# JohannesErnst/WeaSAL

Measured on AMD Instinct MI355X. Metric: points/sec fwd+bwd KPFCNN on DALES spheres; achieved HBM GB/s on KPConv gather, higher is better.
Workload: dtype f32; 1 GPU; DALES_PseudoLabel KP-FCNN, in_radius=10m, 50k pts/sphere, batch=8, fp32, step = GPU pyramid + fwd + loss + bwd + SGD; contrast_loss term included (trainer_PseudoLabel.py:204-208); pyramid of the next batch overlapped on a second stream; parallelism=dp1, dist_world_size=1, allreduce_bytes=0

## Files before the change

### weasal_amd/csrc/contrast_mfma.hip

```cpp
#include "ws_common.h"

namespace {

typedef float f32x4v __attribute__((ext_vector_type(4)));
constexpr int CM_SMAX = 1024;
constexpr float CM_TMIN = 0.023f, CM_TMAX = 1.0e26f;
constexpr int CM_CP = 17;

__device__ __forceinline__ void lds_order()
{
    asm volatile("s_waitcnt lgkmcnt(0)" ::: "memory");
    __builtin_amdgcn_wave_barrier();
}

constexpr int CF_TILES = 2;
constexpr int CF_WAVES = 8;

template <int NS>
__global__ __launch_bounds__(512) void contrast_fwd_mfma_kernel(const float* __restrict__ on, int64_t n, int c,
                                                                 const float* __restrict__ xs, int s,
                                                                 const int64_t* __restrict__ slc_idx, const uint8_t* __restrict__ certain,
                                                                 const int64_t* __restrict__ lbl, float temperature, float eps,
                                                                 float* __restrict__ loss, float* __restrict__ rowmax,
                                                                 float* __restrict__ den, float* __restrict__ npos)
{
    __shared__ float sx[CM_SMAX][4 * NS];
    __shared__ int sidx[CM_SMAX], stag[CM_SMAX];
    const int ncol = (s + 15) & ~15;
    for (int e = threadIdx.x; e < ncol * 4 * NS; e += 512) {
        const int j = e / (4 * NS), cc = e % (4 * NS);
        sx[j][cc] = (j < s && cc < c) ? xs[(int64_t)j * c + cc] : 0.0f;
    }
    for (int j = threadIdx.x; j < ncol; j += 512) {
        const int64_t p = j < s ? slc_idx[j] : 0;
        sidx[j] = j < s ? (int)p : -1;
        stag[j] = j < s ? (((int)lbl[p] << 1) | (certain[p] ? 1 : 0)) : -2;
    }
    __syncthreads();
    const int wave = threadIdx.x >> 6, lane = threadIdx.x & 63;
    const int i = lane & 15, kk = lane >> 4;
    const float inv_t = 1.0f / temperature;
    for (int t = 0; t < CF_TILES; ++t) {
        const int64_t p0 = (((int64_t)blockIdx.x * CF_WAVES + wave) * CF_TILES + t) * 16;
        if (p0 >= n) break;
        float a[NS];
        {
            const int64_t pi = p0 + i < n ? p0 + i : n - 1;
#pragma unroll
            for (int st = 0; st < NS; ++st) a[st] = (4 * st + kk) < c ? on[pi * c + 4 * st + kk] : 0.0f;
        }
        int ptag[4], pidx[4];
        float m[4], E[4], P[4], S[4];
#pragma unroll
        for (int r = 0; r < 4; ++r) {
            const int64_t p = p0 + 4 * kk + r;
            const int64_t pc = p < n ? p : n - 1;
            pidx[r] = (int)p;
            ptag[r] = ((int)lbl[pc] << 1) | (certain[pc] ? 1 : 0);
            m[r] = -3.0e38f; E[r] = 0.0f; P[r] = 0.0f; S[r] = 0.0f;
        }
        for (int c0 = 0; c0 < ncol; c0 += 16) {
            f32x4v d = f32x4v{0.f, 0.f, 0.f, 0.f};
#pragma unroll
            for (int st = 0; st < NS; ++st) d = __builtin_amdgcn_mfma_f32_16x16x4f32(a[st], sx[c0 + i][4 * st + kk], d, 0, 0, 0);
            const int tg = stag[c0 + i], sid = sidx[c0 + i];
            const bool colok = tg != -2;
#pragma unroll
            for (int r = 0; r < 4; ++r) {
                const float mul = d[r] * inv_t;
                m[r] = colok ? fmaxf(m[r], mul) : m[r];
                const bool use = colok && sid != pidx[r] && ((tg ^ ptag[r]) & 1) == 0;
                const bool pos = use && tg == ptag[r];
                E[r] += use ? __expf(mul - inv_t) : 0.0f;
                P[r] += pos ? 1.0f : 0.0f;
                S[r] += pos ? mul : 0.0f;
            }
        }
#pragma unroll
        for (int r = 0; r < 4; ++r) {
#pragma unroll
            for (int o = 1; o < 16; o <<= 1) {
                m[r] = fmaxf(m[r], __shfl_xor(m[r], o, 64));
                E[r] += __shfl_xor(E[r], o, 64);
                P[r] += __shfl_xor(P[r], o, 64);
                S[r] += __shfl_xor(S[r], o, 64);
            }
            const int64_t p = p0 + 4 * kk + r;
            if (i == 0 && p < n) {
                const float Er = E[r] * __expf(inv_t - m[r]);
                const float dd = Er + eps;
                loss[p] = -temperature * (((S[r] - P[r] * m[r]) - P[r] * logf(dd)) / (P[r] + 1e-12f));
                rowmax[p] = m[r];
                den[p] = dd;
                npos[p] = P[r];
            }
        }
    }
}

constexpr int CB_TILES = 4;
constexpr int CB_WLD = 17;

template <int NS>
__global__ __launch_bounds__(256) void contrast_bwd_mfma_kernel(const float* __restrict__ on, int64_t n, int c,
                                                                 const float* __restrict__ xs, int s,
                                                                 const int64_t* __restrict__ slc_idx, const uint8_t* __restrict__ certain,
                                                                 const int64_t* __restrict__ lbl, float temperature,
                                                                 const float* __restrict__ rowmax, const float* __restrict__ den,
                                                                 const float* __restrict__ npos, const float* __restrict__ g,
                                                                 float* __restrict__ d_on, float* __restrict__ partial)
{
    __shared__ float po_all[4][16 * CB_TILES][CM_CP];
    __shared__ float4 pst_all[4][16 * CB_TILES];
    __shared__ int ptg_all[4][16 * CB_TILES];
    __shared__ float wt_all[4][16 * CB_WLD];
    __shared__ float ds_all[4][16][16];
    const int wave = threadIdx.x >> 6, lane = threadIdx.x & 63;
    const int i = lane & 15, kk = lane >> 4;
    float (*po)[CM_CP] = po_all[wave];
    float4* pst = pst_all[wave];
    int* ptg = ptg_all[wave];
    float* wt = wt_all[wave];
    const int64_t pw0 = ((int64_t)blockIdx.x * 4 + wave) * (16 * CB_TILES);
    const float inv_t = 1.0f / temperature;
    for (int e = lane; e < 16 * CB_TILES * CM_CP; e += 64) {
        const int r = e / CM_CP, cc = e % CM_CP;
        const int64_t p = pw0 + r;
        po[r][cc] = (p < n && cc < c) ? on[p * c + cc] : 0.0f;
    }
    for (int r = lane; r < 16 * CB_TILES; r += 64) {
        const int64_t p = pw0 + r;
        const bool live = p < n;
        const float P = live ? npos[p] : 0.0f;
        pst[r] = make_float4(live ? rowmax[p] : 0.0f, P, live ? 1.0f / den[p] : 0.0f,
                             live ? g[p] * (-temperature / (P + 1e-12f)) / temperature : 0.0f);
        ptg[r] = live ? (((int)lbl[p] << 1) | (certain[p] ? 1 : 0)) : -4;
    }
    lds_order();
    f32x4v don[CB_TILES];
#pragma unroll
    for (int t = 0; t < CB_TILES; ++t) don[t] = f32x4v{0.f, 0.f, 0.f, 0.f};
    const int ncol = (s + 15) & ~15;
    for (int c0 = 0; c0 < ncol; c0 += 16) {
        float b1[NS], b2[4];
        const int col = c0 + i;
        const int colc = col < s ? col : s - 1;
#pragma unroll
        for (int st = 0; st < NS; ++st) b1[st] = (col < s && 4 * st + kk < c) ? xs[(int64_t)colc * c + 4 * st + kk] : 0.0f;
#pragma unroll
        for (int st = 0; st < 4; ++st) {
            const int cj = c0 + 4 * st + kk;
            b2[st] = (cj < s && i < c) ? xs[(int64_t)cj * c + i] : 0.0f;
        }
        const int64_t sp = slc_idx[colc];
        const int sid = col < s ? (int)sp : -1;
        const int tg = col < s ? (((int)lbl[sp] << 1) | (certain[sp] ? 1 : 0)) : -2;
        f32x4v dsa = f32x4v{0.f, 0.f, 0.f, 0.f};
#pragma unroll
        for (int t = 0; t < CB_TILES; ++t) {
            f32x4v d = f32x4v{0.f, 0.f, 0.f, 0.f};
#pragma unroll
            for (int st = 0; st < NS; ++st) d = __builtin_amdgcn_mfma_f32_16x16x4f32(po[16 * t + i][4 * st + kk], b1[st], d, 0, 0, 0);
            lds_order();
#pragma unroll
            for (int r = 0; r < 4; ++r) {
                const int pr = 16 * t + 4 * kk + r;
                const float4 st4 = pst[pr];
                const int ptag = ptg[pr];
                const float lg = d[r] * inv_t - st4.x;
                const bool use = tg != -2 && ptag != -4 && sid != (int)(pw0 + pr) && ((tg ^ ptag) & 1) == 0;
                const bool pos = use && tg == ptag;
                const float w = st4.w * ((pos ? 1.0f : 0.0f) - (use ? st4.y * __expf(lg) * st4.z : 0.0f));
                wt[(4 * kk + r) * CB_WLD + i] = w;
            }
            lds_order();
#pragma unroll
            for (int st = 0; st < 4; ++st) {
                don[t] = __builtin_amdgcn_mfma_f32_16x16x4f32(wt[i * CB_WLD + 4 * st + kk], b2[st], don[t], 0, 0, 0);
                dsa = __builtin_amdgcn_mfma_f32_16x16x4f32(po[16 * t + 4 * st + kk][i], wt[(4 * st + kk) * CB_WLD + i], dsa, 0, 0, 0);
            }
        }
#pragma unroll
        for (int r = 0; r < 4; ++r) ds_all[wave][4 * kk + r][i] = dsa[r];
        __syncthreads();
        {
            const int ch = threadIdx.x >> 4, cj = threadIdx.x & 15;
            if (ch < c && c0 + cj < s)
                partial[((int64_t)blockIdx.x * s + c0 + cj) * c + ch] = (ds_all[0][ch][cj] + ds_all[1][ch][cj]) + (ds_all[2][ch][cj] + ds_all[3][ch][cj]);
        }
        __syncthreads();
    }
#pragma unroll
    for (int t = 0; t < CB_TILES; ++t)
#pragma unroll
        for (int r = 0; r < 4; ++r) {
            const int64_t p = pw0 + 16 * t + 4 * kk + r;
            if (p < n && i < c) d_on[p * c + i] = don[t][r];
        }
}

__global__ __launch_bounds__(1024) void contrast_reduce2_kernel(const float* __restrict__ partial, int64_t elems, int chunks,
                                                                 float* __restrict__ out)
{
    __shared__ float red[32][33];
    const int el = threadIdx.x & 31, cl = threadIdx.x >> 5;
    const int64_t e = (int64_t)blockIdx.x * 32 + el;
    float sacc = 0.0f;
    if (e < elems)
        for (int cidx = cl; cidx < chunks; cidx += 32) sacc += partial[(int64_t)cidx * elems + e];
    red[cl][el] = sacc;
    __syncthreads();
    for (int o = 16; o > 0; o >>= 1) {
        if (cl < o) red[cl][el] += red[cl + o][el];
        __syncthreads();
    }
    if (cl == 0 && e < elems) out[e] = red[0][el];
}

}

extern "C" {

int ws_contrast_rows_fwd(const float* on, int64_t n, int32_t c, const float* xs, int32_t s, const int64_t* slc_idx,
                         const uint8_t* certain, const int64_t* lbl, float temperature, float eps, float* loss,
                         float* rowmax, float* den, float* npos, void* stream)
{
    WS_REQUIRE(n >= 0 && c >= 1 && s >= 1, "bad sizes n=%lld c=%d s=%d", (long long)n, c, s);
    if (c > 16 || s > CM_SMAX) return ws_fail(WS_ERR_UNSUPPORTED, "contrast rows: c=%d (<= 16) s=%d (<= %d)", c, s, CM_SMAX);
    WS_REQUIRE(temperature >= CM_TMIN && temperature <= CM_TMAX, "contrast rows: temperature %g outside [%g, %g]", (double)temperature, (double)CM_TMIN, (double)CM_TMAX);
    WS_REQUIRE(n < (1ll << 31), "n exceeds int32");
    if (n == 0) return WS_OK;
    WS_REQUIRE(on && xs && slc_idx && certain && lbl && loss && rowmax && den && npos, "NULL argument");
    hipStream_t st = (hipStream_t)stream;
    const unsigned grid = (unsigned)ws_ceil_div(n, CF_WAVES * CF_TILES * 16);
    if (c <= 4) contrast_fwd_mfma_kernel<1><<<grid, 64 * CF_WAVES, 0, st>>>(on, n, c, xs, s, slc_idx, certain, lbl, temperature, eps, loss, rowmax, den, npos);
    else if (c <= 8) contrast_fwd_mfma_kernel<2><<<grid, 64 * CF_WAVES, 0, st>>>(on, n, c, xs, s, slc_idx, certain, lbl, temperature, eps, loss, rowmax, den, npos);
    else if (c <= 12) contrast_fwd_mfma_kernel<3><<<grid, 64 * CF_WAVES, 0, st>>>(on, n, c, xs, s, slc_idx, certain, lbl, temperature, eps, loss, rowmax, den, npos);
    else contrast_fwd_mfma_kernel<4><<<grid, 64 * CF_WAVES, 0, st>>>(on, n, c, xs, s, slc_idx, certain, lbl, temperature, eps, loss, rowmax, den, npos);
    WS_LAUNCH_CHECK();
    return WS_OK;
}

int64_t ws_contrast_rows_bwd_scratch_bytes(int64_t n, int32_t c, int32_t s)
{
    return ws_ceil_div(n > 0 ? n : 1, 4 * CB_TILES * 16) * (int64_t)s * c * (int64_t)sizeof(float);
}

int ws_contrast_rows_bwd(const float* on, int64_t n, int32_t c, const float* xs, int32_t s, const int64_t* slc_idx,
                         const uint8_t* certain, const int64_t* lbl, float temperature, const float* rowmax,
                         const float* den, const float* npos, const float* g, float* d_on, float* d_xs, void* scratch,
                         void* stream)
{
    WS_REQUIRE(n >= 0 && c >= 1 && s >= 1, "bad sizes n=%lld c=%d s=%d", (long long)n, c, s);
    if (c > 16 || s > CM_SMAX) return ws_fail(WS_ERR_UNSUPPORTED, "contrast rows: c=%d (<= 16) s=%d (<= %d)", c, s, CM_SMAX);
    WS_REQUIRE(temperature >= CM_TMIN && temperature <= CM_TMAX, "contrast rows: temperature %g outside [%g, %g]", (double)temperature, (double)CM_TMIN, (double)CM_TMAX);
    WS_REQUIRE(d_xs, "NULL argument");
    hipStream_t st = (hipStream_t)stream;
    if (n == 0) {
        WS_HIP(hipMemsetAsync(d_xs, 0, sizeof(float) * (size_t)s * c, st));
        return WS_OK;
    }
    WS_REQUIRE(on && xs && slc_idx && certain && lbl && rowmax && den && npos && g && d_on && scratch, "NULL argument");
    const int chunks = (int)ws_ceil_div(n, 4 * CB_TILES * 16);
    float* partial = chunks == 1 ? d_xs : (float*)scratch;
#define WS_CBM(NSV) contrast_bwd_mfma_kernel<NSV><<<chunks, 256, 0, st>>>(on, n, c, xs, s, slc_idx, certain, lbl, temperature, rowmax, den, npos, g, d_on, partial)
    if (c <= 4) WS_CBM(1);
    else if (c <= 8) WS_CBM(2);
    else if (c <= 12) WS_CBM(3);
    else WS_CBM(4);
#undef WS_CBM
    WS_LAUNCH_CHECK();
    if (chunks > 1) {
        const int64_t elems = (int64_t)s * c;
        contrast_reduce2_kernel<<<(unsigned)ws_ceil_div(elems, 32), 1024, 0, st>>>(partial, elems, chunks, d_xs);
        WS_LAUNCH_CHECK();
    }
    return WS_OK;
}

}
```

Baseline: 32.61 million points/s.

## Partition contrast slice columns by certainty to skip masked work in forward kernel

Result: no change. 32.63 million points/s (median of 2 runs) (+0.1%).

```diff
diff --git a/weasal_amd/csrc/contrast_mfma.hip b/weasal_amd/csrc/contrast_mfma.hip
--- a/weasal_amd/csrc/contrast_mfma.hip
+++ b/weasal_amd/csrc/contrast_mfma.hip
@@ -4,8 +4,11 @@
 
 typedef float f32x4v __attribute__((ext_vector_type(4)));
 constexpr int CM_SMAX = 1024;
+constexpr int CM_STAB = CM_SMAX + 16;
 constexpr float CM_TMIN = 0.023f, CM_TMAX = 1.0e26f;
 constexpr int CM_CP = 17;
+constexpr int CM_NTAG = 64;
+constexpr float CM_LOG2E = 1.44269504088896340736f;
 
 __device__ __forceinline__ void lds_order()
 {
@@ -13,35 +16,145 @@
     __builtin_amdgcn_wave_barrier();
 }
 
+struct SliceGroups { int nc, nc16, ntot; };
+
+template <int NT, typename Mark>
+__device__ __forceinline__ SliceGroups stage_slice_meta(int s, const int64_t* __restrict__ slc_idx, const uint8_t* __restrict__ certain,
+                                                         const int64_t* __restrict__ lbl, int* sorig, int* stag, int* sidx,
+                                                         int* chunk_cnt, Mark mark)
+{
+    static_assert(CM_SMAX % NT == 0 && NT % 64 == 0, "whole 64-column chunks per round");
+    constexpr int ROUNDS = CM_SMAX / NT, NCHUNK = CM_SMAX / 64;
+    const int lane = threadIdx.x & 63;
+    const unsigned long long below = (1ull << lane) - 1ull;
+    int pnt[ROUNDS], tag[ROUNDS];
+    unsigned long long cmask[ROUNDS];
+#pragma unroll
+    for (int r = 0; r < ROUNDS; ++r) {
+        const int j = r * NT + (int)threadIdx.x;
+        const bool live = j < s;
+        const int64_t p = live ? slc_idx[j] : 0;
+        pnt[r] = (int)p;
+        tag[r] = live ? (((int)lbl[p] << 1) | (certain[p] ? 1 : 0)) : -2;
+        cmask[r] = __ballot(live && (tag[r] & 1));
+        if (lane == 0) chunk_cnt[j >> 6] = __popcll(cmask[r]);
+    }
+    __syncthreads();
+    int nc = 0;
+#pragma unroll
+    for (int k = 0; k < NCHUNK; ++k) nc += chunk_cnt[k];
+    nc = __builtin_amdgcn_readfirstlane(nc);
+    SliceGroups gr;
+    gr.nc = nc;
+    gr.nc16 = (nc + 15) & ~15;
+    const int nu = s - nc;
+    gr.ntot = gr.nc16 + ((nu + 15) & ~15);
+#pragma unroll
+    for (int r = 0; r < ROUNDS; ++r) {
+        const int j = r * NT + (int)threadIdx.x;
+        if (j < s) {
+            const int k = j >> 6;
+            int before = 0;
+            for (int q = 0; q < k; ++q) before += chunk_cnt[q];
+            const int cb = __popcll(cmask[r] & below);
+            const int pos = (tag[r] & 1) ? before + cb : gr.nc16 + (64 * k - before) + (lane - cb);
+            sorig[pos] = j;
+            stag[pos] = tag[r];
+            sidx[pos] = pnt[r];
+            mark(pos, pnt[r], tag[r]);
+        }
+    }
+    if (threadIdx.x < 32) {
+        const int q = threadIdx.x & 15;
+        const int pos = threadIdx.x < 16 ? nc + q : gr.nc16 + nu + q;
+        if (pos < (threadIdx.x < 16 ? gr.nc16 : gr.ntot)) {
+            sorig[pos] = -1;
+            stag[pos] = -2;
+            sidx[pos] = -1;
+        }
+    }
+    __syncthreads();
+    return gr;
+}
+
 constexpr int CF_TILES = 2;
 constexpr int CF_WAVES = 8;
+static_assert(CF_TILES * CF_WAVES <= 32, "one self bit per point tile of the workgroup");
+
+template <bool FAST>
+__device__ __forceinline__ void contrast_fwd_tile(const f32x4v d, const int tg, const int sid, const int (&ptag)[4], const int (&pidx)[4],
+                                                  const float k1, const float top, float (&m)[4], float (&E)[4], float (&P)[4], float (&S)[4])
+{
+    const bool colok = tg != -2;
+#pragma unroll
+    for (int r = 0; r < 4; ++r) {
+        const float e = __builtin_amdgcn_exp2f(__builtin_fmaf(d[r], k1, -k1));
+        if (FAST) {
+            m[r] = __builtin_amdgcn_fmed3f(m[r], d[r], top);
+            E[r] += e;
+            S[r] += tg == ptag[r] ? d[r] : 0.0f;
+        } else {
+            m[r] = colok ? fmaxf(m[r], d[r]) : m[r];
+            const bool use = colok && sid != pidx[r] && ((tg ^ ptag[r]) & 1) == 0;
+            const bool pos = use && tg == ptag[r];
+            E[r] += use ? e : 0.0f;
+            P[r] += pos ? 1.0f : 0.0f;
+            S[r] += pos ? d[r] : 0.0f;
+        }
+    }
+}
 
 template <int NS>
-__global__ __launch_bounds__(512) void contrast_fwd_mfma_kernel(const float* __restrict__ on, int64_t n, int c,
+__global__ __launch_bounds__(64 * CF_WAVES) void contrast_fwd_mfma_kernel(const float* __restrict__ on, int64_t n, int c,
                                                                  const float* __restrict__ xs, int s,
                                                                  const int64_t* __restrict__ slc_idx, const uint8_t* __restrict__ certain,
                                                                  const int64_t* __restrict__ lbl, float temperature, float eps,
                                                                  float* __restrict__ loss, float* __restrict__ rowmax,
                                                                  float* __restrict__ den, float* __restrict__ npos)
 {
-    __shared__ float sx[CM_SMAX][4 * NS];
-    __shared__ int sidx[CM_SMAX], stag[CM_SMAX];
-    const int ncol = (s + 15) & ~15;
-    for (int e = threadIdx.x; e < ncol * 4 * NS; e += 512) {
-        const int j = e / (4 * NS), cc = e % (4 * NS);
-        sx[j][cc] = (j < s && cc < c) ? xs[(int64_t)j * c + cc] : 0.0f;
-    }
-    for (int j = threadIdx.x; j < ncol; j += 512) {
-        const int64_t p = j < s ? slc_idx[j] : 0;
-        sidx[j] = j < s ? (int)p : -1;
-        stag[j] = j < s ? (((int)lbl[p] << 1) | (certain[p] ? 1 : 0)) : -2;
+    constexpr int NT = 64 * CF_WAVES;
+    __shared__ float sx[CM_STAB][4 * NS];
+    __shared__ int sidx[CM_STAB], stag[CM_STAB], sorig[CM_STAB];
+    __shared__ int chunk_cnt[CM_SMAX / 64], tagcnt[CM_NTAG], flags[2];
+    if (threadIdx.x < CM_NTAG) tagcnt[threadIdx.x] = 0;
+    if (threadIdx.x < 2) flags[threadIdx.x] = 0;
+    const int64_t blk0 = (int64_t)blockIdx.x * (CF_WAVES * CF_TILES * 16);
+    const SliceGroups gr = stage_slice_meta<NT>(s, slc_idx, certain, lbl, sorig, stag, sidx, chunk_cnt,
+        [&](int, int pnt, int tag) {
+            const int64_t rel = (int64_t)pnt - blk0;
+            if (rel >= 0 && rel < CF_WAVES * CF_TILES * 16) atomicOr(&flags[0], 1 << (int)(rel >> 4));
+            if (tag >= 0 && tag < CM_NTAG) atomicAdd(&tagcnt[tag], 1);
+            else atomicOr(&flags[1], 1);
+        });
+    const int total = gr.ntot * 4 * NS;
+    for (int e0 = threadIdx.x; e0 < total; e0 += NT * 8) {
+        float v[8];
+#pragma unroll
+        for (int u = 0; u < 8; ++u) {
+            const int e = e0 + u * NT < total ? e0 + u * NT : total - 1;
+            const int j = e / (4 * NS), cc = e % (4 * NS);
+            const int o = sorig[j];
+            v[u] = xs[(int64_t)(o > 0 ? o : 0) * c + (cc < c ? cc : c - 1)];
+        }
+#pragma unroll
+        for (int u = 0; u < 8; ++u) {
+            const int e = e0 + u * NT;
+            if (e < total) {
+                const int j = e / (4 * NS), cc = e % (4 * NS);
+                sx[j][cc] = (sorig[j] >= 0 && cc < c) ? v[u] : 0.0f;
+            }
+        }
     }
     __syncthreads();
     const int wave = threadIdx.x >> 6, lane = threadIdx.x & 63;
     const int i = lane & 15, kk = lane >> 4;
     const float inv_t = 1.0f / temperature;
+    const float k1 = inv_t * CM_LOG2E;
+    const float top = temperature >= CM_TMIN ? __builtin_inff() : 0.0f;
+    const int nu = s - gr.nc;
     for (int t = 0; t < CF_TILES; ++t) {
-        const int64_t p0 = (((int64_t)blockIdx.x * CF_WAVES + wave) * CF_TILES + t) * 16;
+        const int tb = wave * CF_TILES + t;
+        const int64_t p0 = blk0 + tb * 16;
         if (p0 >= n) break;
         float a[NS];
         {
@@ -50,49 +163,53 @@
             for (int st = 0; st < NS; ++st) a[st] = (4 * st + kk) < c ? on[pi * c + 4 * st + kk] : 0.0f;
         }
         int ptag[4], pidx[4];
-        float m[4], E[4], P[4], S[4];
+        float m[4], Ec[4], Eu[4], P[4], S[4];
 #pragma unroll
         for (int r = 0; r < 4; ++r) {
             const int64_t p = p0 + 4 * kk + r;
             const int64_t pc = p < n ? p : n - 1;
             pidx[r] = (int)p;
             ptag[r] = ((int)lbl[pc] << 1) | (certain[pc] ? 1 : 0);
-            m[r] = -3.0e38f; E[r] = 0.0f; P[r] = 0.0f; S[r] = 0.0f;
-        }
-        for (int c0 = 0; c0 < ncol; c0 += 16) {
-            f32x4v d = f32x4v{0.f, 0.f, 0.f, 0.f};
-#pragma unroll
-            for (int st = 0; st < NS; ++st) d = __builtin_amdgcn_mfma_f32_16x16x4f32(a[st], sx[c0 + i][4 * st + kk], d, 0, 0, 0);
-            const int tg = stag[c0 + i], sid = sidx[c0 + i];
-            const bool colok = tg != -2;
-#pragma unroll
-            for (int r = 0; r < 4; ++r) {
-                const float mul = d[r] * inv_t;
-                m[r] = colok ? fmaxf(m[r], mul) : m[r];
-                const bool use = colok && sid != pidx[r] && ((tg ^ ptag[r]) & 1) == 0;
-                const bool pos = use && tg == ptag[r];
-                E[r] += use ? __expf(mul - inv_t) : 0.0f;
-                P[r] += pos ? 1.0f : 0.0f;
-                S[r] += pos ? mul : 0.0f;
-            }
-        }
+            m[r] = -3.0e38f; Ec[r] = 0.0f; Eu[r] = 0.0f; P[r] = 0.0f; S[r] = 0.0f;
+        }
+        const bool flagged = __builtin_amdgcn_readfirstlane((int)(((flags[0] >> tb) & 1) != 0 || flags[1] != 0)) != 0;
+        auto run_group = [&](const int c_lo, const int c_hi, const int cnt, float (&Eg)[4]) {
+            const int c_fast = flagged ? c_lo : c_hi - ((cnt & 15) ? 16 : 0);
+            for (int c0 = c_lo; c0 < c_fast; c0 += 16) {
+                f32x4v d = f32x4v{0.f, 0.f, 0.f, 0.f};
+#pragma unroll
+                for (int st = 0; st < NS; ++st) d = __builtin_amdgcn_mfma_f32_16x16x4f32(a[st], sx[c0 + i][4 * st + kk], d, 0, 0, 0);
+                contrast_fwd_tile<true>(d, stag[c0 + i], 0, ptag, pidx, k1, top, m, Eg, P, S);
+            }
+            for (int c0 = c_fast; c0 < c_hi; c0 += 16) {
+                f32x4v d = f32x4v{0.f, 0.f, 0.f, 0.f};
+#pragma unroll
+                for (int st = 0; st < NS; ++st) d = __builtin_amdgcn_mfma_f32_16x16x4f32(a[st], sx[c0 + i][4 * st + kk], d, 0, 0, 0);
+                contrast_fwd_tile<false>(d, stag[c0 + i], sidx[c0 + i], ptag, pidx, k1, top, m, Eg, P, S);
+            }
+        };
+        run_group(0, gr.nc16, gr.nc, Ec);
+        run_group(gr.nc16, gr.ntot, nu, Eu);
 #pragma unroll
         for (int r = 0; r < 4; ++r) {
+            float Er = (ptag[r] & 1) ? Ec[r] : Eu[r];
 #pragma unroll
             for (int o = 1; o < 16; o <<= 1) {
                 m[r] = fmaxf(m[r], __shfl_xor(m[r], o, 64));
-                E[r] += __shfl_xor(E[r], o, 64);
+                Er += __shfl_xor(Er, o, 64);
                 P[r] += __shfl_xor(P[r], o, 64);
                 S[r] += __shfl_xor(S[r], o, 64);
             }
             const int64_t p = p0 + 4 * kk + r;
             if (i == 0 && p < n) {
-                const float Er = E[r] * __expf(inv_t - m[r]);
+                const float mr = m[r] * inv_t, Sr = S[r] * inv_t;
+                const float Pr = flagged ? P[r] : ((ptag[r] >= 0 && ptag[r] < CM_NTAG) ? (float)tagcnt[ptag[r]] : 0.0f);
+                Er *= __expf(inv_t - mr);
                 const float dd = Er + eps;
-                loss[p] = -temperature * (((S[r] - P[r] * m[r]) - P[r] * logf(dd)) / (P[r] + 1e-12f));
-                rowmax[p] = m[r];
+                loss[p] = -temperature * (((Sr - Pr * mr) - Pr * logf(dd)) / (Pr + 1e-12f));
+                rowmax[p] = mr;
                 den[p] = dd;
-                npos[p] = P[r];
+                npos[p] = Pr;
             }
         }
     }
```
